# OpenVisualCloud/SVT-HEVC

Measured on AMD Instinct MI355X. Metric: front-half fps, 4K 8-bit encMode 7 random-access B pictures (BASELINE configs[2]): pictures per second through upload + picture preparation + open-loop motion estimation of 2040 LCUs against 2 list(s) (HME L0 64x32 + L1, full-pel 16x9 85-PU search, sub-pel, bi-prediction) + open-loop intra search + , higher is better.
Workload: dtype u8; 1 GPU

## Files before the change

### include/svt_hevc_amd.h

```cpp
#ifndef SVT_HEVC_AMD_H
#define SVT_HEVC_AMD_H

#include <stdint.h>
#include <stddef.h>

#ifdef __cplusplus
extern "C" {
#endif

#define SVT_AMD_API __attribute__((visibility("default")))

typedef enum SvtAmdStatus {
    SVT_AMD_OK = 0,
    SVT_AMD_ERR_BAD_PARAM = -1,
    SVT_AMD_ERR_RESOURCES = -2,
    SVT_AMD_ERR_DEVICE = -3
} SvtAmdStatus;


#define SVT_AMD_LCU_SIZE 64
#define SVT_AMD_ME_PU_COUNT 85
#define SVT_AMD_PAD_FULL 68
#define SVT_AMD_PAD_QUARTER 32
#define SVT_AMD_PAD_SIXTEENTH 16

#define SVT_AMD_SUB_SAD_SEARCH 0
#define SVT_AMD_FULL_SAD_SEARCH 1
#define SVT_AMD_SSD_SEARCH 2

#define SVT_AMD_UNI_PRED_LIST_0 0
#define SVT_AMD_UNI_PRED_LIST_1 1
#define SVT_AMD_BI_PRED 2

typedef struct SvtAmdMeParams {
    uint16_t luma_width;
    uint16_t luma_height;
    uint8_t  num_lists;
    uint8_t  temporal_layer_index;
    uint8_t  ref_pocs_equal;
    uint8_t  enable_hme_flag;
    uint8_t  enable_hme_level0;
    uint8_t  enable_hme_level1;
    uint8_t  enable_hme_level2;
    uint8_t  one_quadrant_hme;
    uint8_t  update_hme_search_center;
    uint8_t  num_hme_regions_w;
    uint8_t  num_hme_regions_h;
    uint8_t  search_area_width;
    uint8_t  search_area_height;
    uint8_t  fractional_search_method;
    uint8_t  fractional_search_model;
    uint8_t  fractional_search_64x64;
    uint8_t  cu8x8_mode;
    uint8_t  cu16x16_mode;
    uint16_t hme_l0_total_w;
    uint16_t hme_l0_total_h;
    uint16_t hme_l0_w[2];
    uint16_t hme_l0_h[2];
    uint16_t hme_l1_w[2];
    uint16_t hme_l1_h[2];
    uint16_t hme_l2_w[2];
    uint16_t hme_l2_h[2];
    uint16_t hme_l0_mult_x;
    uint16_t hme_l0_mult_y;
    uint32_t lambda;
    uint32_t mvd_bits[12];
} SvtAmdMeParams;

typedef struct SvtAmdMeCuResult {
    int16_t  x_mv_l0, y_mv_l0, x_mv_l1, y_mv_l1;
    uint32_t distortion[3];
    uint8_t  direction[3];
    uint8_t  total_me_candidate_index;
} SvtAmdMeCuResult;

typedef struct SvtAmdMeLcuResult {
    SvtAmdMeCuResult pu[SVT_AMD_ME_PU_COUNT];
    uint32_t best_sad[2][SVT_AMD_ME_PU_COUNT];
    uint32_t best_mv[2][SVT_AMD_ME_PU_COUNT];
    int16_t  hme_center_x[2], hme_center_y[2];
    int16_t  search_origin_x[2], search_origin_y[2];
    uint8_t  search_w[2], search_h[2];
} SvtAmdMeLcuResult;


typedef struct SvtAmdContext SvtAmdContext;

SVT_AMD_API int svt_amd_context_create(int device_ordinal, uint16_t max_luma_width,
                                       uint16_t max_luma_height, int num_picture_slots,
                                       SvtAmdContext **out_ctx);
SVT_AMD_API void svt_amd_context_destroy(SvtAmdContext *ctx);
SVT_AMD_API const char *svt_amd_version(void);
SVT_AMD_API int svt_amd_runtime_env_defaults(void);
SVT_AMD_API int svt_amd_host_wait_mode(int device_ordinal, int blocking);
SVT_AMD_API const char *svt_amd_last_error(void);

SVT_AMD_API int svt_amd_picture_upload(SvtAmdContext *ctx, int slot, const uint8_t *luma,
                                       uint32_t stride, uint16_t width, uint16_t height);

SVT_AMD_API int svt_amd_picture_upload_device(SvtAmdContext *ctx, int slot, const void *d_luma,
                                              uint32_t stride, uint16_t width, uint16_t height);
SVT_AMD_API int svt_amd_picture_upload_device_batch(SvtAmdContext *ctx, int num, const int *slots,
                                                    const void *const *d_luma, uint32_t stride,
                                                    uint16_t width, uint16_t height);

SVT_AMD_API int svt_amd_me_picture(SvtAmdContext *ctx, const SvtAmdMeParams *params,
                                   int cur_slot, const int ref_slot[2],
                                   SvtAmdMeLcuResult *out);

SVT_AMD_API int svt_amd_me_picture_launch(SvtAmdContext *ctx, const SvtAmdMeParams *params,
                                          int cur_slot, const int ref_slot[2]);
SVT_AMD_API int svt_amd_me_picture_fetch(SvtAmdContext *ctx, int cur_slot, SvtAmdMeLcuResult *out);
typedef struct SvtAmdMeJob {
    SvtAmdMeParams params;
    int32_t cur_slot;
    int32_t ref_slot[2];
} SvtAmdMeJob;
SVT_AMD_API int svt_amd_me_batch_launch(SvtAmdContext *ctx, const SvtAmdMeJob *jobs, int num_jobs);

SVT_AMD_API int svt_amd_me_picture_range_launch(SvtAmdContext *ctx, const SvtAmdMeParams *params,
                                                int cur_slot, const int ref_slot[2],
                                                uint32_t lcu_begin, uint32_t lcu_end);
SVT_AMD_API int svt_amd_synchronize(SvtAmdContext *ctx);
SVT_AMD_API int svt_amd_device_alloc(SvtAmdContext *ctx, size_t bytes, void **d_ptr);
SVT_AMD_API int svt_amd_device_free(SvtAmdContext *ctx, void *d_ptr);
SVT_AMD_API int svt_amd_device_copy(SvtAmdContext *ctx, void *d_dst, const void *d_src, size_t bytes);
SVT_AMD_API int svt_amd_device_upload(SvtAmdContext *ctx, void *d_dst, const void *src, size_t bytes);
SVT_AMD_API int svt_amd_device_download(SvtAmdContext *ctx, void *dst, const void *d_src, size_t bytes);

typedef struct SvtAmdOisParams {
    uint16_t luma_width, luma_height;
    uint8_t  slice_is_intra;
    uint8_t  temporal_layer_index;
    uint8_t  limit_ois_to_dc_mode;
    uint8_t  skip_ois_8x8;
    uint8_t  cu8x8_mode;
    uint8_t  ois_kernel_level;
    uint8_t  ois_th_set;
    uint8_t  set_best_ois_distortion_to_valid;
} SvtAmdOisParams;

#define SVT_AMD_OIS_MAX_CAND 18
#define SVT_AMD_OIS_W_DIST  (1u << 21)
#define SVT_AMD_OIS_W_VALID (1u << 22)
#define SVT_AMD_OIS_W_MODE  (1u << 23)
typedef struct SvtAmdOisLcuResult {
    uint32_t candidate[SVT_AMD_ME_PU_COUNT][SVT_AMD_OIS_MAX_CAND];
    uint8_t  total_intra_luma_mode[SVT_AMD_ME_PU_COUNT];
    uint8_t  pad[3];
} SvtAmdOisLcuResult;
SVT_AMD_API int svt_amd_ois_picture(SvtAmdContext *ctx, const SvtAmdOisParams *params, int cur_slot,
                                    const SvtAmdMeLcuResult *me, SvtAmdOisLcuResult *out);
SVT_AMD_API int svt_amd_ois_picture_launch(SvtAmdContext *ctx, const SvtAmdOisParams *params, int cur_slot);
SVT_AMD_API int svt_amd_ois_picture_fetch(SvtAmdContext *ctx, int cur_slot, SvtAmdOisLcuResult *out);
typedef struct SvtAmdZzLcu {
    uint32_t sad;
    uint8_t  zz_cost;
    uint8_t  non_moving_index;
    uint8_t  pad[2];
} SvtAmdZzLcu;
SVT_AMD_API int svt_amd_zz_sad_picture(SvtAmdContext *ctx, int cur_slot, int prev_slot, SvtAmdZzLcu *out);

typedef struct SvtAmdFrontendJob {
    int32_t cur_slot;
    int32_t ref_slot[2];
    uint8_t has_me;
    uint8_t has_ois;
    uint8_t compact;
    uint8_t pad;
    SvtAmdMeParams me;
    SvtAmdOisParams ois;
} SvtAmdFrontendJob;
SVT_AMD_API int svt_amd_context_fork(SvtAmdContext *parent, SvtAmdContext **out_lane);
SVT_AMD_API int svt_amd_picture_upload_async(SvtAmdContext *lane, int slot, const uint8_t *luma, uint32_t stride,
                                             uint16_t width, uint16_t height);
SVT_AMD_API int svt_amd_picture_publish(SvtAmdContext *lane, int slot);
SVT_AMD_API int svt_amd_frontend_submit(SvtAmdContext *lane, const SvtAmdFrontendJob *job);
SVT_AMD_API int svt_amd_frontend_wait(SvtAmdContext *lane, const SvtAmdMeLcuResult **me, const SvtAmdOisLcuResult **ois);
SVT_AMD_API int svt_amd_frontend_release(SvtAmdContext *lane);
SVT_AMD_API int svt_amd_lane_event_record(SvtAmdContext *lane, int index);
SVT_AMD_API int svt_amd_lane_event_wait(SvtAmdContext *lane, SvtAmdContext *source, int index);
#define SVT_AMD_OIS_COMPACT_BYTES(nc) (SVT_AMD_ME_PU_COUNT * (nc) * 4 + 88)
SVT_AMD_API int svt_amd_ois_compact_candidates(const SvtAmdOisParams *params);
SVT_AMD_API int svt_amd_me_picture_fetch_compact_async(SvtAmdContext *ctx, int cur_slot, SvtAmdMeCuResult *out);
SVT_AMD_API int svt_amd_ois_picture_fetch_compact_async(SvtAmdContext *ctx, int cur_slot, int candidates, void *out);
SVT_AMD_API int svt_amd_records_pack_batch_async(SvtAmdContext *ctx, const int *slots, int n, int candidates, SvtAmdMeCuResult *d_me,
                                                 void *d_ois);
SVT_AMD_API int svt_amd_frontend_warmup(SvtAmdContext *ctx);
SVT_AMD_API int svt_amd_device_upload_async(SvtAmdContext *ctx, void *d_dst, const void *src, size_t bytes);
SVT_AMD_API int svt_amd_device_download_async(SvtAmdContext *ctx, void *dst, const void *d_src, size_t bytes);
SVT_AMD_API int svt_amd_host_alloc(SvtAmdContext *ctx, size_t bytes, void **h_ptr);
SVT_AMD_API int svt_amd_host_free(SvtAmdContext *ctx, void *h_ptr);
SVT_AMD_API int svt_amd_host_register(SvtAmdContext *ctx, const void *h_ptr, size_t bytes);
SVT_AMD_API int svt_amd_host_unregister_all(SvtAmdContext *ctx);
SVT_AMD_API int svt_amd_me_picture_fetch_async(SvtAmdContext *ctx, int cur_slot, SvtAmdMeLcuResult *out);
SVT_AMD_API int svt_amd_ois_picture_fetch_async(SvtAmdContext *ctx, int cur_slot, SvtAmdOisLcuResult *out);

typedef struct SvtAmdRect { uint16_t x, y, w, h; } SvtAmdRect;
typedef struct SvtAmdCommId { char bytes[128]; } SvtAmdCommId;
SVT_AMD_API int svt_amd_tile_partition(uint16_t luma_width, uint16_t luma_height, int tile_cols, int tile_rows, int world,
                                       SvtAmdRect *rank_rect, int *tile_rank);
SVT_AMD_API int svt_amd_comm_unique_id(SvtAmdCommId *out);
SVT_AMD_API int svt_amd_comm_init(SvtAmdContext *ctx, int world, int rank, const SvtAmdCommId *id);
SVT_AMD_API int svt_amd_comm_destroy(SvtAmdContext *ctx);
SVT_AMD_API int svt_amd_recon_exchange(SvtAmdContext *ctx, void *const d_planes[3], const uint32_t pitch_bytes[3], int bytes_per_sample,
                                       const SvtAmdRect *rects, int world, int rank);
SVT_AMD_API int svt_amd_recon_pack(SvtAmdContext *ctx, void *const d_planes[3], const uint32_t pitch_bytes[3], int bytes_per_sample,
                                   const SvtAmdRect *rects, int world, int r, void *d_slots, size_t slot_bytes, int to_slot);

typedef struct SvtAmdPaLcuStats {
    uint16_t variance[SVT_AMD_ME_PU_COUNT];
    uint8_t y_mean[SVT_AMD_ME_PU_COUNT];
    uint8_t pad;
} SvtAmdPaLcuStats;
SVT_AMD_API int svt_amd_picture_stats(SvtAmdContext *ctx, int slot, SvtAmdPaLcuStats *out, int regions_w, int regions_h, uint32_t *histogram,
                                      uint8_t *region_average, uint64_t *sum_luma);

SVT_AMD_API int svt_amd_picture_ac_energy(SvtAmdContext *ctx, int slot, uint64_t *out);

typedef struct SvtAmdOisJob {
    SvtAmdOisParams params;
    int32_t cur_slot;
} SvtAmdOisJob;
SVT_AMD_API int svt_amd_ois_batch_launch(SvtAmdContext *ctx, const SvtAmdOisJob *jobs, int num_jobs);

typedef struct SvtAmdSideJob {
    int32_t cur_slot;
    int32_t prev_slot;
    uint8_t want_block_stats, want_ac_energy, want_histogram, pad;
} SvtAmdSideJob;
typedef struct SvtAmdSideArrays {
    SvtAmdPaLcuStats *block_stats;
    uint64_t         *ac_energy;
    SvtAmdZzLcu      *zz;
    uint32_t         *histogram;
    uint8_t          *region_average;
    uint64_t         *sum_luma;
} SvtAmdSideArrays;
SVT_AMD_API int svt_amd_side_stats_batch_launch(SvtAmdContext *ctx, const SvtAmdSideJob *jobs, int num_jobs, int regions_w, int regions_h,
                                                const SvtAmdSideArrays *out);
#define SVT_AMD_SIDE_BLOCK_STATS 0
#define SVT_AMD_SIDE_AC_ENERGY   1
#define SVT_AMD_SIDE_ZZ          2
#define SVT_AMD_SIDE_HISTOGRAM   3
#define SVT_AMD_SIDE_REGION_AVG  4
#define SVT_AMD_SIDE_SUM_LUMA    5
SVT_AMD_API size_t svt_amd_side_stats_bytes(uint16_t luma_width, uint16_t luma_height, int which, int regions_w, int regions_h);

typedef struct SvtAmdPaLcuChroma {
    uint8_t cb_mean[21];
    uint8_t cr_mean[21];
    uint8_t pad[6];
} SvtAmdPaLcuChroma;
typedef struct SvtAmdChromaJob {
    const uint8_t *cb, *cr;
    uint32_t pitch;
    uint8_t want_means, want_histogram, pad[2];
} SvtAmdChromaJob;
typedef struct SvtAmdChromaArrays {
    SvtAmdPaLcuChroma *means;
    uint32_t          *histogram;
    uint8_t           *region_average;
    uint64_t          *sum_chroma;
} SvtAmdChromaArrays;
SVT_AMD_API int svt_amd_chroma_stats_batch_launch(SvtAmdContext *ctx, const SvtAmdChromaJob *jobs, int num_jobs, uint16_t luma_width, uint16_t luma_height,
                                                  int regions_w, int regions_h, const SvtAmdChromaArrays *out);
#define SVT_AMD_CHROMA_MEANS      0
#define SVT_AMD_CHROMA_HISTOGRAM  1
#define SVT_AMD_CHROMA_REGION_AVG 2
#define SVT_AMD_CHROMA_SUM        3
SVT_AMD_API size_t svt_amd_chroma_stats_bytes(uint16_t luma_width, uint16_t luma_height, int which, int regions_w, int regions_h);

typedef struct SvtAmdPaLcuDetect {
    uint64_t var_of_var_32x32[4];
    uint16_t edge_cu;
    uint8_t  homogeneous;
    uint8_t  edge_block_num;
    uint8_t  isolated_high_intensity;
    uint8_t  sharp_edge;
    uint8_t  pad[10];
} SvtAmdPaLcuDetect;
typedef struct SvtAmdPaPicDetect {
    uint16_t pic_avg_variance;
    uint8_t  very_low_var_pic;
    uint8_t  logo_pic;
    uint8_t  lcu_block_percentage;
    uint8_t  pad[3];
} SvtAmdPaPicDetect;
typedef struct SvtAmdDetectJob {
    const SvtAmdPaLcuStats  *stats;
    const SvtAmdPaLcuChroma *chroma;
    uint8_t want_edge16, resolution_class, pad[6];
} SvtAmdDetectJob;
typedef struct SvtAmdDetectArrays {
    SvtAmdPaLcuDetect *lcu;
    SvtAmdPaPicDetect *picture;
} SvtAmdDetectArrays;
SVT_AMD_API int svt_amd_picture_detect_batch_launch(SvtAmdContext *ctx, const SvtAmdDetectJob *jobs, int num_jobs, uint16_t luma_width, uint16_t luma_height,
                                                    const SvtAmdDetectArrays *out);
#define SVT_AMD_DETECT_LCU     0
#define SVT_AMD_DETECT_PICTURE 1
SVT_AMD_API size_t svt_amd_picture_detect_bytes(uint16_t luma_width, uint16_t luma_height, int which);

#define SVT_AMD_NOISE_HALF    0
#define SVT_AMD_NOISE_QUARTER 1
#define SVT_AMD_NOISE_FULL    2
typedef struct SvtAmdNoiseJob {
    int32_t cur_slot;
    uint8_t method;
    uint8_t noise_detection_th;
    uint8_t pad[2];
} SvtAmdNoiseJob;
typedef struct SvtAmdNoisePic {
    uint64_t noise_variance_sum;
    uint32_t block_count;
    uint8_t  pic_noise_class;
    uint8_t  pad[3];
} SvtAmdNoisePic;
typedef struct SvtAmdNoiseArrays {
    uint8_t        *flat_noise;
    SvtAmdNoisePic *picture;
} SvtAmdNoiseArrays;
SVT_AMD_API int svt_amd_noise_detect_batch_launch(SvtAmdContext *ctx, const SvtAmdNoiseJob *jobs, int num_jobs, const SvtAmdNoiseArrays *out);
#define SVT_AMD_NOISE_FLAT    0
#define SVT_AMD_NOISE_PICTURE 1
SVT_AMD_API size_t svt_amd_noise_detect_bytes(uint16_t luma_width, uint16_t luma_height, int which);

typedef struct SvtAmdSboJob {
    const SvtAmdPaLcuStats   *stats;
    const SvtAmdPaLcuStats   *ref_stats;
    const SvtAmdPaLcuChroma  *chroma;
    const SvtAmdPaLcuDetect  *detect;
    const uint32_t           *histogram;
    const SvtAmdZzLcu        *zz[17];
    const SvtAmdMeLcuResult  *me;
    const SvtAmdOisLcuResult *ois;
    int32_t cur_slot;
    uint8_t zz_count, slice_type, temporal_layer_index, is_used_as_reference;
    uint8_t resolution_class, skip_ois_8x8, cu8x8_mode, want_qpm;
    uint8_t pad[4];
} SvtAmdSboJob;
typedef struct SvtAmdSboLcu {
    uint16_t grass, skin, high_luma, high_chroma;
    uint8_t  zz_cost, non_moving_index;
    uint8_t  similar_colocated;
    uint8_t  similar_colocated_all_layers;
    uint8_t  failing_motion;
    uint8_t  uncovered_area;
    uint8_t  cmplx_contrast;
    uint8_t  isolated_non_homogeneous;
    uint8_t  cmplx_status;
    uint8_t  complex_lcu;
    uint8_t  pad[6];
} SvtAmdSboLcu;
typedef struct SvtAmdSboPic {
    uint32_t complete_lcu_count;
    uint32_t zz_cost_average;
    uint16_t non_moving_index_average;
    uint8_t  low_motion_content;
    uint8_t  dark_background_light_foreground;
    uint8_t  intra_coded_block_probability;
    uint8_t  grass_percentage;
    uint8_t  percentage_of_edge_in_light_background;
    uint8_t  high_dark_area_density;
    uint8_t  high_dark_low_light_area_density;
    uint8_t  black_area_percentage;
    uint8_t  pad[6];
    uint32_t intra_complexity_min[4], intra_complexity_max[4], intra_complexity_accum[4], intra_complexity_avg[4];
    uint32_t inter_complexity_min[4], inter_complexity_max[4], inter_complexity_accum[4], inter_complexity_avg[4];
    uint32_t processed_leaf_count[4];
} SvtAmdSboPic;
typedef struct SvtAmdSboArrays {
    SvtAmdSboLcu *lcu;
    SvtAmdSboPic *picture;
} SvtAmdSboArrays;
SVT_AMD_API int svt_amd_source_ops_batch_launch(SvtAmdContext *ctx, const SvtAmdSboJob *jobs, int num_jobs, uint16_t luma_width, uint16_t luma_height,
                                                int regions_w, int regions_h, const SvtAmdSboArrays *out);
#define SVT_AMD_SBO_LCU     0
#define SVT_AMD_SBO_PICTURE 1
SVT_AMD_API size_t svt_amd_source_ops_bytes(uint16_t luma_width, uint16_t luma_height, int which);

#define SVT_AMD_MDC_MAX_LCUS 13854
typedef struct SvtAmdMdcJob {
    const SvtAmdMeLcuResult *me;
    const SvtAmdPaLcuStats  *stats;
    const SvtAmdPaLcuDetect *detect;
    const SvtAmdSboLcu      *sbo_lcu;
    const SvtAmdSboPic      *sbo_pic;
    const SvtAmdPaPicDetect *pic_detect;
    const SvtAmdNoisePic    *noise_pic;
    const uint8_t           *stationary_edge;
    int32_t cur_slot;
    uint8_t slice_type;
    uint8_t temporal_layer_index;
    uint8_t hierarchical_levels;
    uint8_t is_used_as_reference;
    uint8_t depth_mode;
    uint8_t enc_mode;
    uint8_t resolution_class;
    uint8_t qp;
    uint8_t is_pan, is_tilt;
    uint8_t noise_detection_th;
    uint8_t homogeneity_percentage;
    uint8_t frame_rate_30;
    uint8_t cu8x8_mode;
    uint8_t average_intensity;
    uint8_t ref_average_intensity[2];
    uint8_t ref_intra_coded_area[2];
    uint8_t ref_temporal_layer[2];
    uint8_t ref_penalize_skip[2];
    uint8_t pad;
    uint32_t lambda_sad;
    uint32_t split_flag_bits[2];
} SvtAmdMdcJob;
typedef struct SvtAmdMdcLcu {
    uint8_t  leaf_count;
    uint8_t  leaf_index[SVT_AMD_ME_PU_COUNT], leaf_split[SVT_AMD_ME_PU_COUNT];
    uint8_t  lcu_md_mode;
    uint8_t  aura_status;
    uint8_t  pred64;
    uint8_t  avc_partitioning;
    uint8_t  pad0;
    uint32_t lcu_score;
    uint8_t  lcu_cost;
    uint8_t  pad[3];
} SvtAmdMdcLcu;
typedef struct SvtAmdMdcPic {
    uint8_t  scene_characteristic_id;
    uint8_t  adjust_min_qp;
    uint8_t  high_intra_selection;
    int8_t   slice_cb_qp_offset, slice_cr_qp_offset;
    int8_t   tc_offset, beta_offset;
    uint8_t  average_qp;
    uint8_t  adp_depth_sensitive_picture_class;
    uint8_t  adp_refinement_mode;
    uint8_t  number_of_segments;
    uint8_t  pad0;
    uint32_t budget;
    uint32_t predicted_cost;
    uint32_t lcu_min_score, lcu_max_score;
    int8_t   score_th[7];
    uint8_t  interval_cost[7];
    uint8_t  iterations;
    uint8_t  bdp_present, md_present;
    uint8_t  pad[3];
} SvtAmdMdcPic;
typedef struct SvtAmdMdcArrays {
    SvtAmdMdcLcu *lcu;
    SvtAmdMdcPic *picture;
} SvtAmdMdcArrays;
SVT_AMD_API int svt_amd_md_config_batch_launch(SvtAmdContext *ctx, const SvtAmdMdcJob *jobs, int num_jobs, uint16_t luma_width, uint16_t luma_height,
                                               const SvtAmdMdcArrays *out);
#define SVT_AMD_MDC_LCU     0
#define SVT_AMD_MDC_PICTURE 1
SVT_AMD_API size_t svt_amd_md_config_bytes(uint16_t luma_width, uint16_t luma_height, int which);
SVT_AMD_API void svt_amd_debug_md_config_stages(int mask);

#define SVT_AMD_IRC_MAX_LCUS 16384
typedef struct SvtAmdIrcChecks {
    uint8_t check1;
    uint8_t pm_check1;
    uint8_t check2;
    uint8_t low_dist_logo;
} SvtAmdIrcChecks;
typedef struct SvtAmdIrcMotion {
    uint32_t total_checked_lcus, total_pan_lcus, total_tilt_lcus, total_pan_high_amp_lcus, total_tilt_high_amp_lcus;
    uint8_t  is_pan_raw, is_tilt_raw;
    uint8_t  pad[2];
} SvtAmdIrcMotion;
typedef struct SvtAmdIrcLcu {
    uint8_t  similar_edge_count[16];
    uint8_t  pm_similar_edge_count[16];
    uint64_t var_of_var_over_time;
    uint8_t  homogeneous_over_time;
    uint8_t  motion_votes;
    uint8_t  pad[6];
} SvtAmdIrcLcu;
typedef struct SvtAmdIrcPic {
    uint8_t  is_pan, is_tilt;
    uint8_t  homogeneity_percentage;
    uint8_t  pad0;
    uint16_t homogeneous_lcu_count;
    uint16_t stationary_lcu_count[4];
    uint8_t  pad[2];
// ... 958 lines not shown
```

### svt-hevc_amd/csrc/prep_kernels.hip

```cpp
#include "svt_amd_internal.h"

__device__ __forceinline__ int clampi(int v, int lo, int hi) { return v < lo ? lo : (v > hi ? hi : v); }
__device__ __forceinline__ uint32_t round_shift_clip(int sum_plus_16)
{
    const uint32_t u = (uint32_t)(sum_plus_16 < 0 ? 0 : sum_plus_16) >> 5;
    return u > 255u ? 255u : u;
}

#define STRIP 16

struct PrepJobDev {
    const uint8_t *raw;
    int32_t raw_stride, w, h;
    uint8_t *full, *quarter, *sixteenth, *B, *H, *J;
    int32_t pitch_full, pitch_quarter, pitch_sixteenth;
};

__device__ __forceinline__ uint32_t vfilt4(uint32_t m2, uint32_t m1, uint32_t c0, uint32_t p1)
{
    uint32_t v = 0;
#pragma unroll
    for (int i = 0; i < 4; i++) {
        const int s = 8 * i;
        v |= round_shift_clip(-2 * (int)((m2 >> s) & 255) + 18 * (int)((m1 >> s) & 255) + 18 * (int)((c0 >> s) & 255) -
                              2 * (int)((p1 >> s) & 255) + 16) << s;
    }
    return v;
}

__device__ __forceinline__ void load7(const uint8_t *row, int x0, int w, bool fast, int (&a)[7], uint32_t &fd)
{
    if (fast) {
        const uint32_t d0 = *(const uint32_t *)(row + x0 - 4), d1 = *(const uint32_t *)(row + x0),
                       d2 = *(const uint32_t *)(row + x0 + 4);
        a[0] = (d0 >> 16) & 255, a[1] = d0 >> 24;
        a[2] = d1 & 255, a[3] = (d1 >> 8) & 255, a[4] = (d1 >> 16) & 255, a[5] = d1 >> 24;
        a[6] = d2 & 255;
        fd = d1;
    } else {
#pragma unroll
        for (int i = 0; i < 7; i++)
            a[i] = row[clampi(x0 - 2 + i, 0, w - 1)];
        fd = (uint32_t)a[2] | ((uint32_t)a[3] << 8) | ((uint32_t)a[4] << 16) | ((uint32_t)a[5] << 24);
    }
}

__global__ __launch_bounds__(256) void k_prep_fused(const PrepJobDev *__restrict__ jobs, int b0, int b1)
{
    const PrepJobDev J = jobs[blockIdx.y];
    const int w = J.w, h = J.h;
    int blk = (int)blockIdx.x;
    if (blk < b0) {
        const int pad = SVT_AMD_PAD_FULL;
        const int cols4 = (w + 2 * pad) >> 2, strips = (h + 2 * pad + STRIP - 1) / STRIP;
        const int g = blk * 256 + (int)threadIdx.x;
        if (g >= cols4 * strips)
            return;
        const int strip = g / cols4, cx = g - strip * cols4;
        const int x0 = -pad + 4 * cx, ys = -pad + STRIP * strip, ye = min(ys + STRIP, h + pad);
        const bool fast = x0 >= 4 && x0 + 8 <= w && ((((uintptr_t)J.raw) | (uint32_t)J.raw_stride) & 3) == 0;
        uint32_t f[4] = {0, 0, 0, 0}, b[4] = {0, 0, 0, 0};
        const ptrdiff_t pf = J.pitch_full;
        for (int r = ys - 2; r <= ye; r++) {
            const uint8_t *row = J.raw + (size_t)clampi(r, 0, h - 1) * J.raw_stride;
            int a[7];
            uint32_t fd, vb = 0;
            load7(row, x0, w, fast, a, fd);
#pragma unroll
            for (int i = 0; i < 4; i++)
                vb |= round_shift_clip(-2 * a[i] + 18 * a[i + 1] + 18 * a[i + 2] - 2 * a[i + 3] + 16) << (8 * i);
            f[0] = f[1], f[1] = f[2], f[2] = f[3], f[3] = fd;
            b[0] = b[1], b[1] = b[2], b[2] = b[3], b[3] = vb;
            if (r >= ys && r < ye) {
                *(uint32_t *)(J.full + r * pf + x0) = fd;
                *(uint32_t *)(J.B + r * pf + x0) = vb;
            }
            const int y = r - 1;
            if (y >= ys && y < ye && r >= ys + 1) {
                *(uint32_t *)(J.H + y * pf + x0) = vfilt4(f[0], f[1], f[2], f[3]);
                *(uint32_t *)(J.J + y * pf + x0) = vfilt4(b[0], b[1], b[2], b[3]);
            }
        }
        return;
    }
    const bool q = blk < b0 + b1;
    blk -= q ? b0 : b0 + b1;
    const int step = q ? 2 : 4, pad = q ? SVT_AMD_PAD_QUARTER : SVT_AMD_PAD_SIXTEENTH;
    const int dw = w / step, dh = h / step;
    uint8_t *dst = q ? J.quarter : J.sixteenth;
    const ptrdiff_t pitch = q ? J.pitch_quarter : J.pitch_sixteenth;
    const int cols4 = (dw + 2 * pad + 3) >> 2, strips = (dh + 2 * pad + 7) / 8;
    const int g = blk * 256 + (int)threadIdx.x;
    if (g >= cols4 * strips)
        return;
    const int strip = g / cols4, cx = g - strip * cols4;
    const int x0 = -pad + 4 * cx, ys = -pad + 8 * strip, ye = min(ys + 8, dh + pad);
    const bool fast = x0 >= 0 && x0 + 4 <= dw && ((((uintptr_t)J.raw) | (uint32_t)J.raw_stride) & (q ? 7 : 15)) == 0;
    for (int y = ys; y < ye; y++) {
        const uint8_t *row = J.raw + (size_t)(clampi(y, 0, dh - 1) * step) * J.raw_stride;
        uint32_t v;
        if (fast && q) {
            const uint2 d = *(const uint2 *)(row + x0 * 2);
            v = __builtin_amdgcn_perm(d.y, d.x, 0x06040200u);
        } else if (fast) {
            const uint4 d = *(const uint4 *)(row + x0 * 4);
            v = (d.x & 255) | ((d.y & 255) << 8) | ((d.z & 255) << 16) | ((d.w & 255) << 24);
        } else {
            v = 0;
#pragma unroll
            for (int i = 0; i < 4; i++)
                v |= (uint32_t)row[clampi(x0 + i, 0, dw - 1) * step] << (8 * i);
        }
        *(uint32_t *)(dst + y * pitch + x0) = v;
    }
}

static_assert(sizeof(PrepJobDev) <= 128, "context.hip reserves 128 bytes per prep descriptor");

int svt_amd_launch_prep_batch(SvtAmdContext *ctx, DevPicture *const *pics, const uint8_t *const *d_luma, uint32_t stride,
                              int n)
{
    static thread_local PrepJobDev host[SVT_AMD_MAX_BATCH];
    const int w = pics[0]->width, h = pics[0]->height;
    for (int i = 0; i < n; i++) {
        const DevPicture *p = pics[i];
        PrepJobDev &j = host[i];
        j.raw = d_luma[i], j.raw_stride = (int)stride, j.w = w, j.h = h;
        j.full = p->full.origin, j.quarter = p->quarter.origin, j.sixteenth = p->sixteenth.origin;
        j.B = p->hp_b.origin, j.H = p->hp_h.origin, j.J = p->hp_j.origin;
        j.pitch_full = p->full.pitch, j.pitch_quarter = p->quarter.pitch, j.pitch_sixteenth = p->sixteenth.pitch;
    }
    const int padf = SVT_AMD_PAD_FULL;
    const int n0 = ((w + 2 * padf) >> 2) * ((h + 2 * padf + STRIP - 1) / STRIP);
    const int n1 = (((w >> 1) + 2 * SVT_AMD_PAD_QUARTER + 3) >> 2) * (((h >> 1) + 2 * SVT_AMD_PAD_QUARTER + 7) / 8);
    const int n2 = (((w >> 2) + 2 * SVT_AMD_PAD_SIXTEENTH + 3) >> 2) * (((h >> 2) + 2 * SVT_AMD_PAD_SIXTEENTH + 7) / 8);
    const int b0 = (n0 + 255) / 256, b1 = (n1 + 255) / 256, b2 = (n2 + 255) / 256;
    int rc = svt_amd_stamp_begin(ctx, KC_PREP);
    if (rc)
        return rc;
    {
        const int rcd = svt_amd_upload_descriptors(ctx, ctx->d_prep_jobs, host, sizeof(PrepJobDev) * (size_t)n);
        if (rcd)
            return rcd;
    }
    hipLaunchKernelGGL(k_prep_fused, dim3(b0 + b1 + b2, n), dim3(256), 0, svt_amd_ctx_stream(ctx), (const PrepJobDev *)ctx->d_prep_jobs, b0, b1);
    HIP_TRY(hipGetLastError());
    return svt_amd_stamp_end(ctx);
}

int svt_amd_launch_prep(SvtAmdContext *ctx, DevPicture *pic, const uint8_t *d_luma, uint32_t stride)
{
    return svt_amd_launch_prep_batch(ctx, &pic, &d_luma, stride, 1);
}
```

Before: 4801 fps.

## Rewrite full-res prep kernel with buffer loads, packed 16-bit filters, aligned wave mapping

Rewrites the full-resolution half-pel prep path. It uses buffer-resource loads and nontemporal stores, packed 16-bit SIMD filter arithmetic built from byte permutes, and a 4-row software-pipelined sliding window with prefetch. Strips are now 32 rows, and waves are mapped so columns align to 256-byte boundaries through a lead offset. It also adds opt-in lane timing marks behind an environment variable. The aim is to cut memory transactions and ALU work in prep, at the cost of more complex boundary handling that may be fragile.

```diff
diff --git a/include/svt_hevc_amd.h b/include/svt_hevc_amd.h
--- a/include/svt_hevc_amd.h
+++ b/include/svt_hevc_amd.h
@@ -180,6 +180,9 @@
 SVT_AMD_API int svt_amd_frontend_release(SvtAmdContext *lane);
 SVT_AMD_API int svt_amd_lane_event_record(SvtAmdContext *lane, int index);
 SVT_AMD_API int svt_amd_lane_event_wait(SvtAmdContext *lane, SvtAmdContext *source, int index);
+SVT_AMD_API int svt_amd_lane_mark(SvtAmdContext *lane, int id);
+SVT_AMD_API int svt_amd_lane_mark_elapsed(SvtAmdContext *from_lane, int from_id, SvtAmdContext *to_lane, int to_id, float *ms);
+SVT_AMD_API int svt_amd_lane_marks_free(SvtAmdContext *lane);
 #define SVT_AMD_OIS_COMPACT_BYTES(nc) (SVT_AMD_ME_PU_COUNT * (nc) * 4 + 88)
 SVT_AMD_API int svt_amd_ois_compact_candidates(const SvtAmdOisParams *params);
 SVT_AMD_API int svt_amd_me_picture_fetch_compact_async(SvtAmdContext *ctx, int cur_slot, SvtAmdMeCuResult *out);
diff --git a/svt-hevc_amd/csrc/lane_marks.hip b/svt-hevc_amd/csrc/lane_marks.hip
--- /dev/null
+++ b/svt-hevc_amd/csrc/lane_marks.hip
@@ -0,0 +1,64 @@
+#include "svt_amd_internal.h"
+#include <stdlib.h>
+#include <mutex>
+#include <unordered_map>
+#include <vector>
+
+static std::mutex g_marks_lock;
+static std::unordered_map<SvtAmdContext *, std::vector<hipEvent_t>> g_marks;
+
+static bool marks_on()
+{
+    static const bool on = getenv("SVT_AMD_LANE_MARKS") != nullptr && atoi(getenv("SVT_AMD_LANE_MARKS")) != 0;
+    return on;
+}
+
+extern "C" int svt_amd_lane_mark(SvtAmdContext *lane, int id)
+{
+    if (!lane || id < 0 || id >= (1 << 20))
+        return SVT_AMD_ERR_BAD_PARAM;
+    if (!marks_on())
+        return SVT_AMD_OK;
+    HIP_TRY(hipSetDevice(lane->device));
+    std::lock_guard<std::mutex> hold(g_marks_lock);
+    std::vector<hipEvent_t> &v = g_marks[lane];
+    if ((size_t)id >= v.size())
+        v.resize((size_t)id + 1, nullptr);
+    if (!v[id])
+        HIP_TRY(hipEventCreate(&v[id]));
+    HIP_TRY(hipEventRecord(v[id], svt_amd_ctx_stream(lane)));
+    return SVT_AMD_OK;
+}
+
+extern "C" int svt_amd_lane_mark_elapsed(SvtAmdContext *from_lane, int from_id, SvtAmdContext *to_lane, int to_id, float *ms)
+{
+    if (!from_lane || !to_lane || !ms || from_id < 0 || to_id < 0 || from_lane->device != to_lane->device)
+        return SVT_AMD_ERR_BAD_PARAM;
+    std::lock_guard<std::mutex> hold(g_marks_lock);
+    const auto a = g_marks.find(from_lane), b = g_marks.find(to_lane);
+    if (a == g_marks.end() || b == g_marks.end() || (size_t)from_id >= a->second.size() || (size_t)to_id >= b->second.size() ||
+        !a->second[from_id] || !b->second[to_id]) {
+        svt_amd_set_error("svt_amd_lane_mark_elapsed: no such mark (is SVT_AMD_LANE_MARKS set?)");
+        return SVT_AMD_ERR_BAD_PARAM;
+    }
+    HIP_TRY(hipSetDevice(from_lane->device));
+    HIP_TRY(hipEventSynchronize(a->second[from_id]));
+    HIP_TRY(hipEventSynchronize(b->second[to_id]));
+    HIP_TRY(hipEventElapsedTime(ms, a->second[from_id], b->second[to_id]));
+    return SVT_AMD_OK;
+}
+
+extern "C" int svt_amd_lane_marks_free(SvtAmdContext *lane)
+{
+    if (!lane)
+        return SVT_AMD_ERR_BAD_PARAM;
+    std::lock_guard<std::mutex> hold(g_marks_lock);
+    const auto it = g_marks.find(lane);
+    if (it == g_marks.end())
+        return SVT_AMD_OK;
+    for (hipEvent_t e : it->second)
+        if (e)
+            (void)hipEventDestroy(e);
+    g_marks.erase(it);
+    return SVT_AMD_OK;
+}
diff --git a/svt-hevc_amd/csrc/prep_kernels.hip b/svt-hevc_amd/csrc/prep_kernels.hip
--- a/svt-hevc_amd/csrc/prep_kernels.hip
+++ b/svt-hevc_amd/csrc/prep_kernels.hip
@@ -1,13 +1,7 @@
 #include "svt_amd_internal.h"
 
 __device__ __forceinline__ int clampi(int v, int lo, int hi) { return v < lo ? lo : (v > hi ? hi : v); }
-__device__ __forceinline__ uint32_t round_shift_clip(int sum_plus_16)
-{
-    const uint32_t u = (uint32_t)(sum_plus_16 < 0 ? 0 : sum_plus_16) >> 5;
-    return u > 255u ? 255u : u;
-}
-
-#define STRIP 16
+#define STRIP 32
 
 struct PrepJobDev {
     const uint8_t *raw;
@@ -16,70 +10,151 @@
     int32_t pitch_full, pitch_quarter, pitch_sixteenth;
 };
 
-__device__ __forceinline__ uint32_t vfilt4(uint32_t m2, uint32_t m1, uint32_t c0, uint32_t p1)
-{
-    uint32_t v = 0;
-#pragma unroll
-    for (int i = 0; i < 4; i++) {
-        const int s = 8 * i;
-        v |= round_shift_clip(-2 * (int)((m2 >> s) & 255) + 18 * (int)((m1 >> s) & 255) + 18 * (int)((c0 >> s) & 255) -
-                              2 * (int)((p1 >> s) & 255) + 16) << s;
-    }
-    return v;
-}
-
-__device__ __forceinline__ void load7(const uint8_t *row, int x0, int w, bool fast, int (&a)[7], uint32_t &fd)
-{
-    if (fast) {
-        const uint32_t d0 = *(const uint32_t *)(row + x0 - 4), d1 = *(const uint32_t *)(row + x0),
-                       d2 = *(const uint32_t *)(row + x0 + 4);
-        a[0] = (d0 >> 16) & 255, a[1] = d0 >> 24;
-        a[2] = d1 & 255, a[3] = (d1 >> 8) & 255, a[4] = (d1 >> 16) & 255, a[5] = d1 >> 24;
-        a[6] = d2 & 255;
-        fd = d1;
-    } else {
-#pragma unroll
-        for (int i = 0; i < 7; i++)
-            a[i] = row[clampi(x0 - 2 + i, 0, w - 1)];
-        fd = (uint32_t)a[2] | ((uint32_t)a[3] << 8) | ((uint32_t)a[4] << 16) | ((uint32_t)a[5] << 24);
-    }
-}
-
-__global__ __launch_bounds__(256) void k_prep_fused(const PrepJobDev *__restrict__ jobs, int b0, int b1)
+typedef unsigned short u16x2 __attribute__((ext_vector_type(2)));
+typedef short i16x2 __attribute__((ext_vector_type(2)));
+__device__ __forceinline__ uint32_t filt_pk(uint32_t a, uint32_t b, uint32_t c, uint32_t d)
+{
+    const u16x2 k9 = {9, 9}, k8 = {8, 8}, k255 = {255, 255};
+    const i16x2 zero = {0, 0};
+    const u16x2 t = (__builtin_bit_cast(u16x2, b) + __builtin_bit_cast(u16x2, c)) * k9 + k8 -
+                    (__builtin_bit_cast(u16x2, a) + __builtin_bit_cast(u16x2, d));
+    const i16x2 s = __builtin_elementwise_max(__builtin_bit_cast(i16x2, t), zero);
+    const u16x2 u = __builtin_elementwise_min((u16x2)(__builtin_bit_cast(u16x2, s) >> 4), k255);
+    return __builtin_bit_cast(uint32_t, u);
+}
+__device__ __forceinline__ uint32_t pack_pk(uint32_t lo, uint32_t hi) { return __builtin_amdgcn_perm(hi, lo, 0x06040200u); }
+
+struct RowPk {
+    uint32_t f01, f23, b01, b23;
+};
+
+#define PREP_RSRC_FLAGS 0x00020000
+#define PREP_STORE_NT 2
+
+template <bool ALIGNED> struct PrepStrip {
+    __amdgpu_buffer_rsrc_t rF, rB, rH, rJ;
+    const uint8_t *raw;
+    size_t rs;
+    uint32_t pf, xo, col[7], sel1, sel01, sel12, sel56;
+    int w, h, ys, rows;
+    RowPk win[4];
+    uint32_t nx[4][3];
+
+    __device__ __forceinline__ void init(const PrepJobDev &J, int cx, int ys_, int ye)
+    {
+        const int pad = SVT_AMD_PAD_FULL, x0 = -pad + 4 * cx;
+        w = J.w, h = J.h, ys = ys_, rows = ye - ys_ + 3;
+        raw = J.raw, rs = (size_t)J.raw_stride, pf = (uint32_t)J.pitch_full, xo = 4u * (uint32_t)cx;
+        const size_t corner = (size_t)pad * pf + pad;
+        const int extent = (int)((uint32_t)(h + 2 * pad - 1) * pf + (uint32_t)(w + 2 * pad));
+        rF = __builtin_amdgcn_make_buffer_rsrc(J.full - corner, 0, extent, PREP_RSRC_FLAGS);
+        rB = __builtin_amdgcn_make_buffer_rsrc(J.B - corner, 0, extent, PREP_RSRC_FLAGS);
+        rH = __builtin_amdgcn_make_buffer_rsrc(J.H - corner, 0, extent, PREP_RSRC_FLAGS);
+        rJ = __builtin_amdgcn_make_buffer_rsrc(J.J - corner, 0, extent, PREP_RSRC_FLAGS);
+        sel1 = 0x03020100u, sel01 = 0x0c030c02u, sel12 = 0x0c040c03u, sel56 = 0x0c040c03u;
+        if (ALIGNED) {
+            const int c0 = x0 - 4, c2 = x0 + 4;
+            col[0] = (uint32_t)clampi(c0, 0, w - 4), col[1] = (uint32_t)clampi(x0, 0, w - 4), col[2] = (uint32_t)clampi(c2, 0, w - 4);
+            const uint32_t m02 = c0 < 0 ? 0u : (c0 >= w ? 3u : 2u), m03 = c0 < 0 ? 0u : 3u;
+            const uint32_t m20 = c2 >= w ? 3u : 0u;
+            sel1 = x0 < 0 ? 0u : (x0 >= w ? 0x03030303u : 0x03020100u);
+            sel01 = 0x0c000c00u | m02 | (m03 << 16);
+            sel12 = 0x0c040c00u | m03;
+            sel56 = 0x0c040c03u + (m20 << 16);
+        } else {
+#pragma unroll
+            for (int i = 0; i < 7; i++)
+                col[i] = (uint32_t)clampi(x0 - 2 + i, 0, w - 1);
+        }
+#pragma unroll
+        for (int k = 0; k < 4; k++) {
+            win[k] = RowPk{0, 0, 0, 0};
+            load(k, k);
+        }
+    }
+    __device__ __forceinline__ void load(int i, int k)
+    {
+        const __amdgpu_buffer_rsrc_t r =
+            __builtin_amdgcn_make_buffer_rsrc((void *)(raw + (size_t)clampi(ys - 2 + i, 0, h - 1) * rs), 0, w, PREP_RSRC_FLAGS);
+        if (ALIGNED) {
+#pragma unroll
+            for (int j = 0; j < 3; j++)
+                nx[k][j] = __builtin_amdgcn_raw_buffer_load_b32(r, (int)col[j], 0, 0);
+        } else {
+            uint32_t a[7];
+#pragma unroll
+            for (int j = 0; j < 7; j++)
+                a[j] = __builtin_amdgcn_raw_buffer_load_b8(r, (int)col[j], 0, 0);
+            nx[k][0] = (a[0] << 16) | (a[1] << 24);
+            nx[k][1] = a[2] | (a[3] << 8) | (a[4] << 16) | (a[5] << 24);
+            nx[k][2] = a[6];
+        }
+    }
+    enum { HEAD, STEADY, TAIL };
+    template <int MODE> __device__ __forceinline__ void group(int i0)
+    {
+#pragma unroll
+        for (int k = 0; k < 4; k++) {
+            const int i = i0 + k;
+            __builtin_amdgcn_sched_barrier(0);
+            const uint32_t fd = __builtin_amdgcn_perm(0u, nx[k][1], sel1);
+            const uint32_t p01 = __builtin_amdgcn_perm(0u, nx[k][0], sel01), p12 = __builtin_amdgcn_perm(fd, nx[k][0], sel12);
+            const uint32_t p23 = __builtin_amdgcn_perm(0u, fd, 0x0c010c00u), p34 = __builtin_amdgcn_perm(0u, fd, 0x0c020c01u);
+            const uint32_t p45 = __builtin_amdgcn_perm(0u, fd, 0x0c030c02u), p56 = __builtin_amdgcn_perm(nx[k][2], fd, sel56);
+            if (MODE != TAIL || i + 4 < rows)
+                load(i + 4, k);
+            __builtin_amdgcn_sched_barrier(0);
+            RowPk &c = win[k];
+            c.f01 = p23, c.f23 = p45;
+            c.b01 = filt_pk(p01, p12, p23, p34), c.b23 = filt_pk(p23, p34, p45, p56);
+            const int so = (int)((uint32_t)(ys + SVT_AMD_PAD_FULL - 2 + i) * pf);
+            if (MODE == STEADY || (MODE == HEAD ? k == 2 || (k == 3 && rows >= 5) : i <= rows - 2)) {
+                __builtin_amdgcn_raw_buffer_store_b32(fd, rF, (int)xo, so, PREP_STORE_NT);
+                __builtin_amdgcn_raw_buffer_store_b32(pack_pk(c.b01, c.b23), rB, (int)xo, so, PREP_STORE_NT);
+            }
+            if (MODE == STEADY || (MODE == HEAD ? k == 3 : i <= rows - 1)) {
+                const RowPk &m1 = win[(k + 3) & 3], &m2 = win[(k + 2) & 3], &m3 = win[(k + 1) & 3];
+                __builtin_amdgcn_raw_buffer_store_b32(
+                    pack_pk(filt_pk(m3.f01, m2.f01, m1.f01, c.f01), filt_pk(m3.f23, m2.f23, m1.f23, c.f23)), rH, (int)xo, so - (int)pf, PREP_STORE_NT);
+                __builtin_amdgcn_raw_buffer_store_b32(
+                    pack_pk(filt_pk(m3.b01, m2.b01, m1.b01, c.b01), filt_pk(m3.b23, m2.b23, m1.b23, c.b23)), rJ, (int)xo, so - (int)pf, PREP_STORE_NT);
+            }
+        }
+    }
+    __device__ __forceinline__ void run()
+    {
+        int i0 = 4;
+        group<HEAD>(0);
+        for (; i0 + 3 <= rows - 2; i0 += 4)
+            group<STEADY>(i0);
+        for (; i0 < rows; i0 += 4)
+            group<TAIL>(i0);
+    }
+};
+
+__global__ __launch_bounds__(256) void k_prep_fused(const PrepJobDev *__restrict__ jobs, int b0, int b1, int lead)
 {
     const PrepJobDev J = jobs[blockIdx.y];
     const int w = J.w, h = J.h;
     int blk = (int)blockIdx.x;
     if (blk < b0) {
         const int pad = SVT_AMD_PAD_FULL;
-        const int cols4 = (w + 2 * pad) >> 2, strips = (h + 2 * pad + STRIP - 1) / STRIP;
-        const int g = blk * 256 + (int)threadIdx.x;
-        if (g >= cols4 * strips)
+        const int cols4 = (w + 2 * pad) >> 2, wps = (cols4 + lead + 63) >> 6, strips = (h + 2 * pad + STRIP - 1) / STRIP;
+        const int gw = __builtin_amdgcn_readfirstlane(blk * 4 + (int)(threadIdx.x >> 6));
+        if (gw >= wps * strips)
             return;
-        const int strip = g / cols4, cx = g - strip * cols4;
-        const int x0 = -pad + 4 * cx, ys = -pad + STRIP * strip, ye = min(ys + STRIP, h + pad);
-        const bool fast = x0 >= 4 && x0 + 8 <= w && ((((uintptr_t)J.raw) | (uint32_t)J.raw_stride) & 3) == 0;
-        uint32_t f[4] = {0, 0, 0, 0}, b[4] = {0, 0, 0, 0};
-        const ptrdiff_t pf = J.pitch_full;
-        for (int r = ys - 2; r <= ye; r++) {
-            const uint8_t *row = J.raw + (size_t)clampi(r, 0, h - 1) * J.raw_stride;
-            int a[7];
-            uint32_t fd, vb = 0;
-            load7(row, x0, w, fast, a, fd);
-#pragma unroll
-            for (int i = 0; i < 4; i++)
-                vb |= round_shift_clip(-2 * a[i] + 18 * a[i + 1] + 18 * a[i + 2] - 2 * a[i + 3] + 16) << (8 * i);
-            f[0] = f[1], f[1] = f[2], f[2] = f[3], f[3] = fd;
-            b[0] = b[1], b[1] = b[2], b[2] = b[3], b[3] = vb;
-            if (r >= ys && r < ye) {
-                *(uint32_t *)(J.full + r * pf + x0) = fd;
-                *(uint32_t *)(J.B + r * pf + x0) = vb;
-            }
-            const int y = r - 1;
-            if (y >= ys && y < ye && r >= ys + 1) {
-                *(uint32_t *)(J.H + y * pf + x0) = vfilt4(f[0], f[1], f[2], f[3]);
-                *(uint32_t *)(J.J + y * pf + x0) = vfilt4(b[0], b[1], b[2], b[3]);
-            }
+        const int strip = gw / wps, cx = (gw - strip * wps) * 64 + (int)(threadIdx.x & 63) - lead;
+        if (cx < 0 || cx >= cols4)
+            return;
+        const int ys = -pad + STRIP * strip, ye = min(ys + STRIP, h + pad);
+        if (((((uintptr_t)J.raw) | (uint32_t)J.raw_stride) & 3) == 0) {
+            PrepStrip<true> s;
+            s.init(J, cx, ys, ye);
+            s.run();
+        } else {
+            PrepStrip<false> s;
+            s.init(J, cx, ys, ye);
+            s.run();
         }
         return;
     }
@@ -131,7 +206,8 @@
         j.pitch_full = p->full.pitch, j.pitch_quarter = p->quarter.pitch, j.pitch_sixteenth = p->sixteenth.pitch;
     }
     const int padf = SVT_AMD_PAD_FULL;
-    const int n0 = ((w + 2 * padf) >> 2) * ((h + 2 * padf + STRIP - 1) / STRIP);
+    const int lead = (int)(((uintptr_t)(pics[0]->full.origin - padf) & 255) >> 2);
+    const int n0 = 64 * ((((w + 2 * padf) >> 2) + lead + 63) >> 6) * ((h + 2 * padf + STRIP - 1) / STRIP);
     const int n1 = (((w >> 1) + 2 * SVT_AMD_PAD_QUARTER + 3) >> 2) * (((h >> 1) + 2 * SVT_AMD_PAD_QUARTER + 7) / 8);
     const int n2 = (((w >> 2) + 2 * SVT_AMD_PAD_SIXTEENTH + 3) >> 2) * (((h >> 2) + 2 * SVT_AMD_PAD_SIXTEENTH + 7) / 8);
     const int b0 = (n0 + 255) / 256, b1 = (n1 + 255) / 256, b2 = (n2 + 255) / 256;
@@ -143,7 +219,7 @@
         if (rcd)
             return rcd;
     }
-    hipLaunchKernelGGL(k_prep_fused, dim3(b0 + b1 + b2, n), dim3(256), 0, svt_amd_ctx_stream(ctx), (const PrepJobDev *)ctx->d_prep_jobs, b0, b1);
+    hipLaunchKernelGGL(k_prep_fused, dim3(b0 + b1 + b2, n), dim3(256), 0, svt_amd_ctx_stream(ctx), (const PrepJobDev *)ctx->d_prep_jobs, b0, b1, lead);
     HIP_TRY(hipGetLastError());
     return svt_amd_stamp_end(ctx);
 }
```

After: 4822 fps (median of 5 runs). No clear change (+0.4%).
